# ait-detectmate/DetectMateService

Hardware: AMD Instinct MI355X
Metric: lines_per_sec (higher is better)
Workload: dtype bf16; 1 GPU; model=matcher_parser+new_value+bert-tiny-detector, global_batch=65536, seq_len=64, max_line_len=256, parallelism=dp1, ingest=shm_ring+proto_decode, transformer=True, hip_graph=False, device=cuda:0

## Files before the change

### detectmateservice_amd/ops/csrc/bert_fused.hip

```cpp
#include "common.h"
#include "kernels.h"

typedef __attribute__((address_space(3))) short lds_short;
typedef __attribute__((address_space(3))) short4v lds_short4;
typedef __attribute__((address_space(3))) float lds_float;
typedef __attribute__((address_space(1))) const short glob_cshort;
typedef __attribute__((address_space(1))) const float glob_cfloat;

#define BF_THREADS (BF_WAVES * DMX_WAVE)

#define XS (BF_H + 8)
#define QKS (2 * BF_H + 16)
#define VTS (BF_S + 8)

extern __shared__ __attribute__((aligned(16))) short smem_raw[];

template <int OFF_, int ROWS, int COLS_, int STRIDE_>
struct Tile {
  static constexpr int OFF = OFF_, COLS = COLS_, STRIDE = STRIDE_;
  static constexpr int END = OFF + ROWS * STRIDE;
  static_assert(OFF % 4 == 0 && STRIDE % 4 == 0 && COLS <= STRIDE,
                "8-byte LDS access: offsets and strides are multiples of 4");
  static __device__ __forceinline__ lds_short* ptr() {
    return (lds_short*)smem_raw + OFF;
  }
};
using XTile = Tile<0, BF_S, BF_H, XS>;
using QkTile = Tile<XTile::END, BF_S, 2 * BF_H, QKS>;
using PTiles = Tile<XTile::END, BF_WAVES * 16, BF_S, VTS>;
using AttnOut = Tile<PTiles::END, BF_S, BF_H, XS>;
using FfnHalf = Tile<XTile::END, BF_S, BF_FFN / 2, QKS>;
using VtTile = Tile<AttnOut::END, 2 * BF_DH, BF_S, VTS>;
using XMid = Tile<VtTile::OFF, BF_S, BF_H, XS>;
constexpr int RED_OFF = VtTile::END;

static_assert(QkTile::END <= VtTile::OFF, "Q|K runs past buf");
static_assert(FfnHalf::END <= VtTile::OFF, "the FFN half runs past buf");
static_assert(PTiles::END <= AttnOut::OFF,
              "the P tiles reach into the attention output");
static_assert(AttnOut::END <= VtTile::OFF,
              "the attention output runs past buf");
static_assert(XMid::END <= VtTile::END, "XMid runs past vt");
static_assert(BF_LDS_BYTES == RED_OFF * sizeof(short) + BF_H * sizeof(float),
              "kernels.h BF_LDS_BYTES out of step with the LDS strides");
static_assert(FB_BQKV % 4 == 0 && FB_BO % 4 == 0 && FB_B1 % 4 == 0 &&
                  FB_B2 % 4 == 0 && FB_SIZE % 4 == 0 &&
                  (BF_FFN / 2) % 4 == 0,
              "16-byte bias loads: bias offsets must be multiples of 4");

struct FragLane {
  int l15, l4;
  __device__ __forceinline__ explicit FragLane(int lane)
      : l15(lane & 15), l4(lane >> 4) {}
};

static __device__ __forceinline__ bf16x8 lds_frag(const lds_short* base,
                                                  int stride, int r0, int k0,
                                                  FragLane fl) {
  return *(const __attribute__((address_space(3))) bf16x8*)(
      base + (r0 + fl.l15) * stride + k0 + fl.l4 * 8);
}

static __device__ __forceinline__ lds_short4* lds_quad(lds_short* base,
                                                       int stride, int r0,
                                                       int c0, FragLane fl) {
  return (lds_short4*)(base + (r0 + fl.l15) * stride + c0 + fl.l4 * 4);
}

typedef __attribute__((ext_vector_type(4))) __bf16 bf16x4_t;
static __device__ __forceinline__ short4v pack_bf16x4(f32x4 v) {
  return __builtin_bit_cast(short4v, __builtin_convertvector(v, bf16x4_t));
}

template <int K, int MODE, int ACT, int WTS, int ABL, bool BIAS, bool SWAP>
static __device__ __forceinline__ void gemm_quad(
    const lds_short* __restrict__ in_lds, int in_stride,
    const glob_cshort* __restrict__ Wt, const glob_cfloat* __restrict__ bias,
    lds_short* __restrict__ out_lds, int out_stride,
    lds_short* __restrict__ x_lds, lds_short* __restrict__ vt_lds, int fn,
    int lane, bf16x8 zb) {
  static_assert(SWAP || MODE == 1, "only the V quads keep weight-as-B order");
  constexpr int KS = K / 32;
  const int l15 = lane & 15;
  const int l4 = lane >> 4;
  f32x4 binit = {0.f, 0.f, 0.f, 0.f};
  if constexpr (BIAS) {
    if constexpr (SWAP) {
      binit = *(const __attribute__((address_space(1))) f32x4*)(bias + fn * 16 +
                                                               l4 * 4);
    } else {
      const float bval = bias[fn * 16 + l15];
      binit = {bval, bval, bval, bval};
    }
  }
  f32x4 acc[4];
#pragma unroll
  for (int i = 0; i < 4; ++i) acc[i] = binit;
#pragma unroll 4
  for (int ks = 0; ks < KS; ++ks) {
    bf16x8 w;
    if constexpr (ABL & 1) {
      w = zb;
    } else {
      w = *(const __attribute__((address_space(1))) bf16x8*)(
          Wt + (long)(fn * 16 + l15) * WTS + ks * 32 + l4 * 8);
    }
#pragma unroll
    for (int fm = 0; fm < 4; ++fm) {
      bf16x8 a;
      if constexpr (ABL & 2) {
        a = zb;
      } else {
        a = *(const __attribute__((address_space(3))) bf16x8*)(
            in_lds + (fm * 16 + l15) * in_stride + ks * 32 + l4 * 8);
      }
      if constexpr (SWAP)
        acc[fm] = __builtin_amdgcn_mfma_f32_16x16x32_bf16(w, a, acc[fm], 0, 0, 0);
      else
        acc[fm] = __builtin_amdgcn_mfma_f32_16x16x32_bf16(a, w, acc[fm], 0, 0, 0);
    }
  }
#pragma unroll
  for (int fm = 0; fm < 4; ++fm) {
    f32x4 v = acc[fm];
    if constexpr (!SWAP) {
      *(lds_short4*)(vt_lds + (fn * 16 + l15 - 2 * BF_H) * VTS + fm * 16 +
                     l4 * 4) = pack_bf16x4(v);
    } else if constexpr (MODE == 2) {
      lds_short4* px = (lds_short4*)(x_lds + (fm * 16 + l15) * XS + fn * 16 + l4 * 4);
      const short4v xv = *px;
#pragma unroll
      for (int r = 0; r < 4; ++r) v[r] += bf16_to_f32(xv[r]);
      *px = pack_bf16x4(v);
    } else if constexpr (MODE == 3) {
      const int off = (fm * 16 + l15) * XS + fn * 16 + l4 * 4;
      const short4v xv = *(const lds_short4*)(x_lds + off);
#pragma unroll
      for (int r = 0; r < 4; ++r) v[r] += bf16_to_f32(xv[r]);
      *(lds_short4*)(out_lds + off) = pack_bf16x4(v);
    } else {
      if constexpr (ACT == 1) {
#pragma unroll
        for (int r = 0; r < 4; ++r) v[r] = gelu_f32(v[r]);
      }
      *(lds_short4*)(out_lds + (fm * 16 + l15) * out_stride + fn * 16 + l4 * 4) =
          pack_bf16x4(v);
    }
  }
}

template <int K, int MODE, int ACT, int WTS, int ABL, bool BIAS, bool SWAP,
          int CNT>
static __device__ __forceinline__ void gemm_quads(
    const lds_short* __restrict__ in_lds, int in_stride,
    const glob_cshort* __restrict__ Wt, const glob_cfloat* __restrict__ bias,
    lds_short* __restrict__ out_lds, int out_stride,
    lds_short* __restrict__ x_lds, lds_short* __restrict__ vt_lds, int fn0,
    int lane, bf16x8 zb) {
#pragma unroll 2
  for (int q = 0; q < CNT; ++q)
    gemm_quad<K, MODE, ACT, WTS, ABL, BIAS, SWAP>(in_lds, in_stride, Wt, bias, out_lds,
                                            out_stride, x_lds, vt_lds, fn0 + q,
                                            lane, zb);
}

template <int K, int N, int MODE, int ACT, int WTS, int ABL = 0,
          bool BIAS = true>
static __device__ __attribute__((noinline)) void block_gemm(
    const lds_short* __restrict__ in_lds, int in_stride,
    const glob_cshort* __restrict__ Wt, const glob_cfloat* __restrict__ bias,
    lds_short* __restrict__ out_lds, int out_stride,
    lds_short* __restrict__ x_lds, lds_short* __restrict__ vt_lds, int wid,
    int lane) {
  bf16x8 zb;
  if constexpr (ABL != 0) {
#pragma unroll
    for (int j = 0; j < 8; ++j) zb[j] = (short)0x3f01;
    asm volatile("" : "+v"(zb));
  }
  constexpr int N16 = N / 16;
  constexpr int TOTAL = 4 * N16;
  constexpr int FPW = TOTAL / BF_WAVES;
  static_assert(FPW >= 4 && FPW % 4 == 0, "quad-chunked assignment");
  constexpr int QPW = FPW / 4;
  const int fn_lo = __builtin_amdgcn_readfirstlane(wid) * QPW;
  if constexpr (MODE != 1) {
    gemm_quads<K, MODE, ACT, WTS, ABL, BIAS, true, QPW>(in_lds, in_stride, Wt, bias,
                                                  out_lds, out_stride, x_lds,
                                                  vt_lds, fn_lo, lane, zb);
  } else {
    constexpr int FN_SWAP = 2 * BF_H / 16;
    constexpr int NSW = FN_SWAP % QPW;
    if (fn_lo + QPW <= FN_SWAP) {
      gemm_quads<K, MODE, ACT, WTS, ABL, BIAS, true, QPW>(in_lds, in_stride, Wt, bias,
                                                    out_lds, out_stride, x_lds,
                                                    vt_lds, fn_lo, lane, zb);
    } else if (fn_lo >= FN_SWAP) {
      gemm_quads<K, MODE, ACT, WTS, ABL, BIAS, false, QPW>(in_lds, in_stride, Wt,
                                                     bias, out_lds, out_stride,
                                                     x_lds, vt_lds, fn_lo, lane,
                                                     zb);
    } else {
      gemm_quads<K, MODE, ACT, WTS, ABL, BIAS, true, NSW>(in_lds, in_stride, Wt, bias,
                                                    out_lds, out_stride, x_lds,
                                                    vt_lds, fn_lo, lane, zb);
      gemm_quads<K, MODE, ACT, WTS, ABL, BIAS, false, QPW - NSW>(
          in_lds, in_stride, Wt, bias, out_lds, out_stride, x_lds, vt_lds,
          fn_lo + NSW, lane, zb);
    }
  }
}

static __device__ __forceinline__ void embed(
    const unsigned char* __restrict__ lines, const int* __restrict__ start,
    const int* __restrict__ end, const short* __restrict__ wb, lds_short* x_lds,
    int line, int max_len, int tid) {
  const int s0 = start[line], e0 = end[line];
  for (int i = tid * 8; i < BF_S * BF_H; i += BF_THREADS * 8) {
    const int s = i / BF_H, c = i % BF_H;
    int tok = 0;
    const int idx = s0 + s;
    if (idx < e0 && idx < max_len)
      tok = (int)lines[(long)line * max_len + idx] + 3;
    short8v te = *(const short8v*)(wb + WB_TOK + (long)tok * BF_H + c);
    short8v pe = *(const short8v*)(wb + WB_POS + (long)s * BF_H + c);
    short8v xv;
#pragma unroll
    for (int j = 0; j < 8; ++j)
      xv[j] = f32_to_bf16(bf16_to_f32(te[j]) + bf16_to_f32(pe[j]));
    *(__attribute__((address_space(3))) short8v*)(x_lds + s * XS + c) = xv;
  }
}

static __device__ __forceinline__ void attention(int wid, int lane) {
  const FragLane fl(lane);
  const int hh = wid >> 2;
  const int q0 = (wid & 3) * 16;
  const float scale = 0.125f;

  f32x4 acc_p[4];
#pragma unroll
  for (int f = 0; f < 4; ++f) acc_p[f] = {0.f, 0.f, 0.f, 0.f};
#pragma unroll
  for (int ks = 0; ks < BF_DH / 32; ++ks) {
    bf16x8 qf = lds_frag(QkTile::ptr(), QKS, q0, hh * BF_DH + ks * 32, fl);
#pragma unroll
    for (int f = 0; f < 4; ++f)
      acc_p[f] = __builtin_amdgcn_mfma_f32_16x16x32_bf16(
          lds_frag(QkTile::ptr(), QKS, f * 16, BF_H + hh * BF_DH + ks * 32, fl),
          qf, acc_p[f], 0, 0, 0);
  }
  float m = -1e30f;
#pragma unroll
  for (int f = 0; f < 4; ++f)
#pragma unroll
    for (int r = 0; r < 4; ++r) m = fmaxf(m, acc_p[f][r] * scale);
  m = fmaxf(m, __shfl_xor(m, 16, 64));
  m = fmaxf(m, __shfl_xor(m, 32, 64));
  float sum = 0.f;
#pragma unroll
  for (int f = 0; f < 4; ++f)
#pragma unroll
    for (int r = 0; r < 4; ++r) {
      const float e = __expf(acc_p[f][r] * scale - m);
      acc_p[f][r] = e;
      sum += e;
    }
  sum += __shfl_xor(sum, 16, 64);
  sum += __shfl_xor(sum, 32, 64);
  const float inv = 1.f / sum;
  __syncthreads();
  lds_short* my_p = PTiles::ptr() + wid * 16 * VTS;
#pragma unroll
  for (int f = 0; f < 4; ++f)
    *lds_quad(my_p, VTS, 0, f * 16, fl) = pack_bf16x4(acc_p[f]);
  asm volatile("s_waitcnt lgkmcnt(0)" ::: "memory");

  f32x4 acc_o[4];
#pragma unroll
  for (int f = 0; f < 4; ++f) acc_o[f] = {0.f, 0.f, 0.f, 0.f};
#pragma unroll
  for (int ks = 0; ks < BF_S / 32; ++ks) {
    bf16x8 pf = lds_frag(my_p, VTS, 0, ks * 32, fl);
#pragma unroll
    for (int f = 0; f < 4; ++f)
      acc_o[f] = __builtin_amdgcn_mfma_f32_16x16x32_bf16(
          lds_frag(VtTile::ptr(), VTS, hh * BF_DH + f * 16, ks * 32, fl), pf,
          acc_o[f], 0, 0, 0);
  }
#pragma unroll
  for (int f = 0; f < 4; ++f) {
    f32x4 o = acc_o[f];
#pragma unroll
    for (int r = 0; r < 4; ++r) o[r] *= inv;
    *lds_quad(AttnOut::ptr(), XS, q0, hh * BF_DH + f * 16, fl) = pack_bf16x4(o);
  }
}

static __device__ __forceinline__ void block_layernorm(
    lds_short* x_lds, const short* __restrict__ gamma,
    const short* __restrict__ beta, int wid, int lane, float eps) {
  const int row = wid * 8 + (lane >> 3);
  const int c0 = (lane & 7) * 16;
  short8v va = *(const __attribute__((address_space(3))) short8v*)(x_lds + row * XS + c0);
  short8v vb = *(const __attribute__((address_space(3))) short8v*)(x_lds + row * XS + c0 + 8);
  float v[16];
  float sum = 0.f;
#pragma unroll
  for (int j = 0; j < 8; ++j) {
    v[j] = bf16_to_f32(va[j]);
    v[8 + j] = bf16_to_f32(vb[j]);
    sum += v[j] + v[8 + j];
  }
#pragma unroll
  for (int mask = 1; mask < 8; mask <<= 1) sum += __shfl_xor(sum, mask, 64);
  const float mean = sum / BF_H;
  float var = 0.f;
#pragma unroll
  for (int j = 0; j < 16; ++j) {
    const float d = v[j] - mean;
    var += d * d;
  }
#pragma unroll
  for (int mask = 1; mask < 8; mask <<= 1) var += __shfl_xor(var, mask, 64);
  const float rstd = rsqrtf(var / BF_H + eps);
  short8v ga = *(const short8v*)(gamma + c0);
  short8v gb = *(const short8v*)(gamma + c0 + 8);
  short8v ba = *(const short8v*)(beta + c0);
  short8v bb = *(const short8v*)(beta + c0 + 8);
  short8v oa, ob;
#pragma unroll
  for (int j = 0; j < 8; ++j) {
    oa[j] = f32_to_bf16((v[j] - mean) * rstd * bf16_to_f32(ga[j]) +
                        bf16_to_f32(ba[j]));
    ob[j] = f32_to_bf16((v[8 + j] - mean) * rstd * bf16_to_f32(gb[j]) +
                        bf16_to_f32(bb[j]));
  }
  *(__attribute__((address_space(3))) short8v*)(x_lds + row * XS + c0) = oa;
  *(__attribute__((address_space(3))) short8v*)(x_lds + row * XS + c0 + 8) = ob;
}

static __device__ __forceinline__ void pool_score(
    const short* __restrict__ w_score, const float* __restrict__ b_score,
    float* __restrict__ score, int tid) {
  const lds_short* x_lds = XTile::ptr();
  lds_float* red = (lds_float*)((lds_short*)smem_raw + RED_OFF);
  if (tid < BF_H) {
    float s = 0.f;
    for (int row = 0; row < BF_S; ++row)
      s += bf16_to_f32(x_lds[row * XS + tid]);
    red[tid] = (s / BF_S) * bf16_to_f32(w_score[tid]);
  }
  __syncthreads();
  const int wid = tid / DMX_WAVE, lane = tid % DMX_WAVE;
  if (wid == 0) {
    float v = red[lane] + red[lane + 64];
    v = warp_reduce_sum_f32(v);
    if (lane == 0) *score = v + *b_score;
  }
}

static __device__ __forceinline__ void pool_embed(
    float* __restrict__ emb, const float* __restrict__ mu,
    const float* __restrict__ inv_var, float* __restrict__ dist, int line,
    int tid) {
  const lds_short* x_lds = XTile::ptr();
  lds_float* red = (lds_float*)((lds_short*)smem_raw + RED_OFF);
  if (tid < BF_H) {
    float s = 0.f;
    for (int row = 0; row < BF_S; ++row)
      s += bf16_to_f32(x_lds[row * XS + tid]);
    const float m = s / BF_S;
    if (emb != nullptr) emb[(long)line * BF_H + tid] = m;
    if (mu != nullptr) {
      const float d = m - mu[tid];
      red[tid] = d * d * inv_var[tid];
    }
  }
  if (mu == nullptr) return;
  __syncthreads();
  const int wid = tid / DMX_WAVE, lane = tid % DMX_WAVE;
  if (wid == 0) {
    float v = red[lane] + red[lane + 64];
    v = warp_reduce_sum_f32(v);
    if (lane == 0) dist[line] = sqrtf(v / BF_H);
  }
}

#define HEAD_SCORE 0
#define HEAD_EMBED 1

#define PH_QKV 1
#define PH_ATTN 2
#define PH_PROJ 4
#define PH_LN 8
#define PH_FFN 16
#define PH_ALL 31

template <bool TIMED>
struct StampRecorder {
  __device__ void mark() {}
  __device__ void flush(unsigned long long*, int, int, int) {}
};
template <>
struct StampRecorder<true> {
  unsigned long long t[BF_NSTAMP];
  int n = 0;
  __device__ void mark() {
    if (n < BF_NSTAMP) t[n++] = __builtin_amdgcn_s_memrealtime();
  }
  __device__ void flush(unsigned long long* out, int line, int wid, int lane) {
    if (lane == 0 && out != nullptr) {
      unsigned long long* dst = out + ((long)line * BF_WAVES + wid) * BF_NSTAMP;
      for (int k = 0; k < BF_NSTAMP; ++k) dst[k] = k < n ? t[k] : 0ull;
    }
  }
};

template <int PHASES, bool TIMED = false, int ABL = 0, int HEAD = HEAD_SCORE>
static __device__ __forceinline__ void bert_fused_body(
    const unsigned char* __restrict__ lines,
    const int* __restrict__ start,
    const int* __restrict__ end,
    const short* __restrict__ wb,
    const float* __restrict__ fb,
    float* __restrict__ scores,
    int B, int max_len, int n_layers, float eps,
    unsigned long long* __restrict__ stamps_out = nullptr,
    float* __restrict__ emb = nullptr,
    const float* __restrict__ mu = nullptr,
    const float* __restrict__ inv_var = nullptr,
    float* __restrict__ dist = nullptr) {
  StampRecorder<TIMED> stamp;
  const int line = blockIdx.x;
  if (line >= B) return;
  const int tid = threadIdx.x;
  const int wid = tid / DMX_WAVE;
  const int lane = tid % DMX_WAVE;

  lds_short* const x = XTile::ptr();

  stamp.mark();
  embed(lines, start, end, wb, x, line, max_len, tid);
  stamp.mark();
  __syncthreads();
  stamp.mark();

  for (int layer = 0; layer < n_layers; ++layer) {
    const short* lw = wb + WB_LAYER0 + (long)layer * LW_SIZE;
    const float* lf = fb + (long)layer * FB_SIZE;

    if (PHASES & PH_QKV)
      block_gemm<BF_H, 3 * BF_H, 1, 0, BF_H, ABL>(x, XS, (glob_cshort*)(lw + LW_QKV),
                                             (glob_cfloat*)(lf + FB_BQKV), QkTile::ptr(), QKS, x, VtTile::ptr(),
                                             wid, lane);
    stamp.mark();
    __syncthreads();
    stamp.mark();

    if (PHASES & PH_ATTN) attention(wid, lane);
    stamp.mark();
    __syncthreads();
    stamp.mark();

    if (PHASES & PH_PROJ)
      block_gemm<BF_H, BF_H, 2, 0, BF_H, ABL>(AttnOut::ptr(), XS, (glob_cshort*)(lw + LW_WO),
                                         (glob_cfloat*)(lf + FB_BO), nullptr, 0, x,
                                         nullptr, wid, lane);
    __syncthreads();
    if (PHASES & PH_LN)
      block_layernorm(x, lw + LW_LN1G, lw + LW_LN1B, wid, lane, eps);
    stamp.mark();
    __syncthreads();
    stamp.mark();

    if (PHASES & PH_FFN)
#pragma unroll
    for (int h = 0; h < 2; ++h) {
      block_gemm<BF_H, BF_FFN / 2, 0, 1, BF_H, ABL>(
          x, XS, (glob_cshort*)(lw + LW_W1 + (long)h * (BF_FFN / 2) * BF_H),
          (glob_cfloat*)(lf + FB_B1 + h * (BF_FFN / 2)), FfnHalf::ptr(), QKS, nullptr,
          nullptr, wid, lane);
      __syncthreads();
      if (h == 0)
        block_gemm<BF_FFN / 2, BF_H, 3, 0, BF_FFN, ABL, true>(
            FfnHalf::ptr(), QKS, (glob_cshort*)(lw + LW_W2), (glob_cfloat*)(lf + FB_B2),
            XMid::ptr(), XS, x, nullptr, wid, lane);
      else
        block_gemm<BF_FFN / 2, BF_H, 3, 0, BF_FFN, ABL, false>(
            FfnHalf::ptr(), QKS, (glob_cshort*)(lw + LW_W2 + (long)h * (BF_FFN / 2)),
            nullptr, x, XS, XMid::ptr(), nullptr, wid, lane);
      __syncthreads();
    }
    if (PHASES & PH_LN)
      block_layernorm(x, lw + LW_LN2G, lw + LW_LN2B, wid, lane, eps);
    stamp.mark();
    __syncthreads();
    stamp.mark();
  }

  if constexpr (HEAD == HEAD_EMBED)
    pool_embed(emb, mu, inv_var, dist, line, tid);
  else
    pool_score(wb + WB_LAYER0 + (long)n_layers * LW_SIZE,
               fb + (long)n_layers * FB_SIZE, scores + line, tid);
  stamp.mark();
  stamp.flush(stamps_out, line, wid, lane);
}

extern "C" __global__ __launch_bounds__(BF_THREADS, 4)
void dmx_bert_fused_bf16(const unsigned char* __restrict__ lines,
                         const int* __restrict__ start,
                         const int* __restrict__ end,
                         const short* __restrict__ wb,
                         const float* __restrict__ fb,
                         float* __restrict__ scores, int B, int max_len,
                         int n_layers, float eps) {
  bert_fused_body<PH_ALL>(lines, start, end, wb, fb, scores, B, max_len,
                          n_layers, eps);
}

extern "C" __global__ __launch_bounds__(BF_THREADS, 4)
void dmx_bert_fused_embed_bf16(const unsigned char* __restrict__ lines,
                               const int* __restrict__ start,
                               const int* __restrict__ end,
                               const short* __restrict__ wb,
                               const float* __restrict__ fb,
                               float* __restrict__ emb,
                               const float* __restrict__ mu,
                               const float* __restrict__ inv_var,
                               float* __restrict__ dist, int B, int max_len,
                               int n_layers, float eps) {
  bert_fused_body<PH_ALL, false, 0, HEAD_EMBED>(lines, start, end, wb, fb,
                                                nullptr, B, max_len, n_layers,
                                                eps, nullptr, emb, mu, inv_var,
                                                dist);
}

template <int PHASES, int ABL = 0>
__global__ __launch_bounds__(BF_THREADS, 4) void dmx_bert_fused_probe(
    const unsigned char* lines, const int* start, const int* end,
    const short* wb, const float* fb, float* scores, int B, int max_len,
    int n_layers, float eps) {
  bert_fused_body<PHASES, false, ABL>(lines, start, end, wb, fb, scores, B,
                                      max_len, n_layers, eps);
}

extern "C" __global__ __launch_bounds__(BF_THREADS, 4)
void dmx_bert_fused_timed(const unsigned char* lines, const int* start,
                          const int* end, const short* wb, const float* fb,
                          float* scores, int B, int max_len, int n_layers,
                          float eps, unsigned long long* stamps) {
  bert_fused_body<PH_ALL, true>(lines, start, end, wb, fb, scores, B,
                                max_len, n_layers, eps, stamps);
}

constexpr int BF_MAX_DEVICES = 64;
typedef bool AttrDone[BF_MAX_DEVICES];

template <typename... KArgs, typename... Args>
static hipError_t launch_bert_fused(void (*kernel)(KArgs...),
                                    AttrDone& attr_done, int B,
                                    hipStream_t stream, Args... args) {
  int dev = 0;
  hipError_t err = hipGetDevice(&dev);
  if (err != hipSuccess) return err;
  if (dev < 0 || dev >= BF_MAX_DEVICES) return hipErrorInvalidDevice;
  if (!attr_done[dev]) {
    err = hipFuncSetAttribute((const void*)kernel,
                              hipFuncAttributeMaxDynamicSharedMemorySize,
                              BF_LDS_BYTES);
    if (err != hipSuccess) return err;
    attr_done[dev] = true;
  }
  hipLaunchKernelGGL(kernel, dim3(B), dim3(BF_THREADS), BF_LDS_BYTES, stream,
                     args...);
  return hipSuccess;
}

extern "C" hipError_t dmx_launch_bert_fused_bf16(
    const uint8_t* lines, const int32_t* start, const int32_t* end,
    const int16_t* wb, const float* fb, float* scores, int B, int max_len,
    int n_layers, float eps, hipStream_t stream) {
  static AttrDone attr_done;
  return launch_bert_fused(dmx_bert_fused_bf16, attr_done, B, stream, lines,
                           start, end, wb, fb, scores, B, max_len, n_layers,
                           eps);
}

extern "C" hipError_t dmx_launch_bert_fused_embed(
    const uint8_t* lines, const int32_t* start, const int32_t* end,
    const int16_t* wb, const float* fb, float* emb, const float* mu,
    const float* inv_var, float* dist, int B, int max_len, int n_layers,
    float eps, hipStream_t stream) {
  static AttrDone attr_done;
  return launch_bert_fused(dmx_bert_fused_embed_bf16, attr_done, B, stream,
                           lines, start, end, wb, fb, emb, mu, inv_var, dist,
                           B, max_len, n_layers, eps);
}

extern "C" hipError_t dmx_launch_bert_fused_timed(
    const uint8_t* lines, const int32_t* start, const int32_t* end,
    const int16_t* wb, const float* fb, float* scores, int64_t* stamps, int B,
    int max_len, int n_layers, float eps, hipStream_t stream) {
  static AttrDone attr_done;
  return launch_bert_fused(dmx_bert_fused_timed, attr_done, B, stream, lines,
                           start, end, wb, fb, scores, B, max_len, n_layers,
                           eps, (unsigned long long*)stamps);
}

struct ProbeVariant {
  int mask;
  decltype(&dmx_bert_fused_probe<0, 0>) kernel;
  AttrDone attr_done;
};
template <int PHASES, int ABL = 0>
constexpr ProbeVariant probe_variant() {
  return {PHASES | (ABL << 8), dmx_bert_fused_probe<PHASES, ABL>, {}};
}
static ProbeVariant probe_variants[] = {
    probe_variant<0>(),
    probe_variant<PH_QKV>(),
    probe_variant<PH_QKV | PH_ATTN>(),
    probe_variant<PH_QKV | PH_ATTN | PH_PROJ>(),
    probe_variant<PH_QKV | PH_ATTN | PH_PROJ | PH_LN>(),
    probe_variant<PH_ALL>(),
    probe_variant<PH_FFN>(),
    probe_variant<PH_LN>(),
    probe_variant<PH_ALL, 1>(),
    probe_variant<PH_ALL, 2>(),
    probe_variant<PH_ALL, 3>(),
    probe_variant<PH_FFN, 1>(),
    probe_variant<PH_FFN, 2>(),
    probe_variant<PH_FFN, 3>(),
};

static ProbeVariant* find_probe_variant(int phase_mask) {
  for (ProbeVariant& v : probe_variants)
    if (v.mask == phase_mask) return &v;
  return nullptr;
}

extern "C" bool dmx_bert_fused_probe_mask_known(int phase_mask) {
  return find_probe_variant(phase_mask) != nullptr;
}

extern "C" hipError_t dmx_launch_bert_fused_probe(
    const uint8_t* lines, const int32_t* start, const int32_t* end,
    const int16_t* wb, const float* fb, float* scores, int B, int max_len,
    int n_layers, float eps, int phase_mask, hipStream_t stream) {
  ProbeVariant* v = find_probe_variant(phase_mask);
  if (v == nullptr) return hipErrorInvalidValue;
  return launch_bert_fused(v->kernel, v->attr_done, B, stream, lines, start,
                           end, wb, fb, scores, B, max_len, n_layers, eps);
}
```

Baseline: 8.571 million lines/s.

## Keep activation fragments stationary in registers across quads for K=128 GEMMs

Adds an activation-stationary GEMM path for the K=128 projections. It loads the 4x4 activation fragments from LDS once per wave and reuses them across all of the wave's output quads, and it prefetches the next quad's weights and bias while the current MFMAs run. By default this is enabled only for the fused QKV GEMM; the W1 path stays on the old routine because its macro defaults to off. The change also re-materialises lane and wave ids per layer to steer register allocation. Holding the fragments costs more VGPRs, which may hurt occupancy under the 4-blocks-per-CU launch bound.

```diff
diff --git a/detectmateservice_amd/ops/csrc/bert_fused.hip b/detectmateservice_amd/ops/csrc/bert_fused.hip
--- a/detectmateservice_amd/ops/csrc/bert_fused.hip
+++ b/detectmateservice_amd/ops/csrc/bert_fused.hip
@@ -162,6 +162,118 @@
     gemm_quad<K, MODE, ACT, WTS, ABL, BIAS, SWAP>(in_lds, in_stride, Wt, bias, out_lds,
                                             out_stride, x_lds, vt_lds, fn0 + q,
                                             lane, zb);
+}
+
+#ifndef BF_ASTAT_QKV
+#define BF_ASTAT_QKV 1
+#endif
+#ifndef BF_ASTAT_W1
+#define BF_ASTAT_W1 0
+#endif
+
+template <int WTS, int ABL>
+static __device__ __forceinline__ bf16x8 astat_wfrag(
+    const glob_cshort* __restrict__ Wt, int fn, int ks, int l15, int l4,
+    bf16x8 zb) {
+  if constexpr (ABL & 1) {
+    return zb;
+  } else {
+    return *(const __attribute__((address_space(1))) bf16x8*)(
+        Wt + (long)(fn * 16 + l15) * WTS + ks * 32 + l4 * 8);
+  }
+}
+
+template <bool SWAP>
+static __device__ __forceinline__ f32x4 astat_bias(
+    const glob_cfloat* __restrict__ bias, int fn, int l15, int l4) {
+  if constexpr (SWAP) {
+    return *(const __attribute__((address_space(1))) f32x4*)(bias + fn * 16 +
+                                                             l4 * 4);
+  } else {
+    const float bval = bias[fn * 16 + l15];
+    return f32x4{bval, bval, bval, bval};
+  }
+}
+
+template <int MODE, int ACT, int WTS, int ABL, int CNT, int NSW, int Q = 0>
+static __device__ __forceinline__ void astat_quads(
+    const bf16x8 (&a)[4][4], bf16x8 (&w)[4], f32x4 binit,
+    const glob_cshort* __restrict__ Wt, const glob_cfloat* __restrict__ bias,
+    lds_short* __restrict__ out_lds, int out_stride,
+    lds_short* __restrict__ vt_lds, int fn0, int lane, bf16x8 zb) {
+  constexpr bool SWAP = Q < NSW;
+  constexpr bool MORE = Q + 1 < CNT;
+  static_assert(SWAP || MODE == 1, "only the V quads keep weight-as-B order");
+  const int l15 = lane & 15;
+  const int l4 = lane >> 4;
+  const int fn = fn0 + Q;
+  f32x4 bnext = {0.f, 0.f, 0.f, 0.f};
+  if constexpr (MORE) bnext = astat_bias<(Q + 1 < NSW)>(bias, fn + 1, l15, l4);
+  f32x4 acc[4];
+#pragma unroll
+  for (int i = 0; i < 4; ++i) acc[i] = binit;
+#pragma unroll
+  for (int ks = 0; ks < 4; ++ks) {
+#pragma unroll
+    for (int fm = 0; fm < 4; ++fm) {
+      if constexpr (SWAP)
+        acc[fm] = __builtin_amdgcn_mfma_f32_16x16x32_bf16(w[ks], a[ks][fm], acc[fm], 0, 0, 0);
+      else
+        acc[fm] = __builtin_amdgcn_mfma_f32_16x16x32_bf16(a[ks][fm], w[ks], acc[fm], 0, 0, 0);
+    }
+    if constexpr (MORE) {
+      w[ks] = astat_wfrag<WTS, ABL>(Wt, fn + 1, ks, l15, l4, zb);
+      __builtin_amdgcn_sched_barrier(0);
+    }
+  }
+#pragma unroll
+  for (int fm = 0; fm < 4; ++fm) {
+    f32x4 v = acc[fm];
+    if constexpr (!SWAP) {
+      *(lds_short4*)(vt_lds + (fn * 16 + l15 - 2 * BF_H) * VTS + fm * 16 +
+                     l4 * 4) = pack_bf16x4(v);
+    } else {
+      if constexpr (ACT == 1) {
+#pragma unroll
+        for (int r = 0; r < 4; ++r) v[r] = gelu_f32(v[r]);
+      }
+      *(lds_short4*)(out_lds + (fm * 16 + l15) * out_stride + fn * 16 + l4 * 4) =
+          pack_bf16x4(v);
+    }
+  }
+  if constexpr (MORE)
+    astat_quads<MODE, ACT, WTS, ABL, CNT, NSW, Q + 1>(
+        a, w, bnext, Wt, bias, out_lds, out_stride, vt_lds, fn0, lane, zb);
+}
+
+template <int MODE, int ACT, int WTS, int ABL, int CNT, int NSW>
+static __device__ __forceinline__ void gemm_quads_astat(
+    const lds_short* __restrict__ in_lds, int in_stride,
+    const glob_cshort* __restrict__ Wt, const glob_cfloat* __restrict__ bias,
+    lds_short* __restrict__ out_lds, int out_stride,
+    lds_short* __restrict__ vt_lds, int fn0, int lane, bf16x8 zb) {
+  const int l15 = lane & 15;
+  const int l4 = lane >> 4;
+  const f32x4 binit = astat_bias<(0 < NSW)>(bias, fn0, l15, l4);
+  bf16x8 w[4];
+#pragma unroll
+  for (int ks = 0; ks < 4; ++ks)
+    w[ks] = astat_wfrag<WTS, ABL>(Wt, fn0, ks, l15, l4, zb);
+  bf16x8 a[4][4];
+#pragma unroll
+  for (int ks = 0; ks < 4; ++ks)
+#pragma unroll
+    for (int fm = 0; fm < 4; ++fm) {
+      if constexpr (ABL & 2) {
+        a[ks][fm] = zb;
+      } else {
+        a[ks][fm] = *(const __attribute__((address_space(3))) bf16x8*)(
+            in_lds + (fm * 16 + l15) * in_stride + ks * 32 + l4 * 8);
+      }
+    }
+  __builtin_amdgcn_sched_barrier(0);
+  astat_quads<MODE, ACT, WTS, ABL, CNT, NSW>(a, w, binit, Wt, bias, out_lds,
+                                             out_stride, vt_lds, fn0, lane, zb);
 }
 
 template <int K, int N, int MODE, int ACT, int WTS, int ABL = 0,
@@ -211,6 +323,51 @@
   }
 }
 
+template <int N, int MODE, int ACT, int ABL>
+static __device__ __forceinline__ void block_gemm_k128(
+    const lds_short* __restrict__ in_lds, int in_stride,
+    const glob_cshort* __restrict__ Wt, const glob_cfloat* __restrict__ bias,
+    lds_short* __restrict__ out_lds, int out_stride,
+    lds_short* __restrict__ vt_lds, int wid, int lane) {
+  static_assert(MODE == 0 || MODE == 1, "the multi-quad K = 128 GEMMs");
+  constexpr int QPW = N / 16 / BF_WAVES;
+  static_assert(QPW > 1 && QPW * 16 * BF_WAVES == N, "whole quads per wave");
+  if constexpr (MODE == 1 ? !BF_ASTAT_QKV : !BF_ASTAT_W1) {
+    block_gemm<BF_H, N, MODE, ACT, BF_H, ABL>(in_lds, in_stride, Wt, bias,
+                                              out_lds, out_stride, nullptr,
+                                              vt_lds, wid, lane);
+  } else {
+    bf16x8 zb;
+    if constexpr (ABL != 0) {
+#pragma unroll
+      for (int j = 0; j < 8; ++j) zb[j] = (short)0x3f01;
+      asm volatile("" : "+v"(zb));
+    }
+    const int fn_lo = __builtin_amdgcn_readfirstlane(wid) * QPW;
+    if constexpr (MODE == 0) {
+      gemm_quads_astat<MODE, ACT, BF_H, ABL, QPW, QPW>(
+          in_lds, in_stride, Wt, bias, out_lds, out_stride, vt_lds, fn_lo, lane,
+          zb);
+    } else {
+      constexpr int FN_SWAP = 2 * BF_H / 16;
+      constexpr int NSW = FN_SWAP % QPW;
+      if (fn_lo + QPW <= FN_SWAP) {
+        gemm_quads_astat<MODE, ACT, BF_H, ABL, QPW, QPW>(
+            in_lds, in_stride, Wt, bias, out_lds, out_stride, vt_lds, fn_lo,
+            lane, zb);
+      } else if (fn_lo >= FN_SWAP) {
+        gemm_quads_astat<MODE, ACT, BF_H, ABL, QPW, 0>(
+            in_lds, in_stride, Wt, bias, out_lds, out_stride, vt_lds, fn_lo,
+            lane, zb);
+      } else {
+        gemm_quads_astat<MODE, ACT, BF_H, ABL, QPW, NSW>(
+            in_lds, in_stride, Wt, bias, out_lds, out_stride, vt_lds, fn_lo,
+            lane, zb);
+      }
+    }
+  }
+}
+
 static __device__ __forceinline__ void embed(
     const unsigned char* __restrict__ lines, const int* __restrict__ start,
     const int* __restrict__ end, const short* __restrict__ wb, lds_short* x_lds,
@@ -435,8 +592,8 @@
   const int line = blockIdx.x;
   if (line >= B) return;
   const int tid = threadIdx.x;
-  const int wid = tid / DMX_WAVE;
-  const int lane = tid % DMX_WAVE;
+  const int wid0 = tid / DMX_WAVE;
+  const int lane0 = tid % DMX_WAVE;
 
   lds_short* const x = XTile::ptr();
 
@@ -449,11 +606,13 @@
   for (int layer = 0; layer < n_layers; ++layer) {
     const short* lw = wb + WB_LAYER0 + (long)layer * LW_SIZE;
     const float* lf = fb + (long)layer * FB_SIZE;
+    int lane = lane0, wid = wid0;
+    asm volatile("" : "+v"(lane), "+v"(wid));
 
     if (PHASES & PH_QKV)
-      block_gemm<BF_H, 3 * BF_H, 1, 0, BF_H, ABL>(x, XS, (glob_cshort*)(lw + LW_QKV),
-                                             (glob_cfloat*)(lf + FB_BQKV), QkTile::ptr(), QKS, x, VtTile::ptr(),
-                                             wid, lane);
+      block_gemm_k128<3 * BF_H, 1, 0, ABL>(x, XS, (glob_cshort*)(lw + LW_QKV),
+                                           (glob_cfloat*)(lf + FB_BQKV), QkTile::ptr(), QKS,
+                                           VtTile::ptr(), wid, lane);
     stamp.mark();
     __syncthreads();
     stamp.mark();
@@ -477,9 +636,9 @@
     if (PHASES & PH_FFN)
 #pragma unroll
     for (int h = 0; h < 2; ++h) {
-      block_gemm<BF_H, BF_FFN / 2, 0, 1, BF_H, ABL>(
+      block_gemm_k128<BF_FFN / 2, 0, 1, ABL>(
           x, XS, (glob_cshort*)(lw + LW_W1 + (long)h * (BF_FFN / 2) * BF_H),
-          (glob_cfloat*)(lf + FB_B1 + h * (BF_FFN / 2)), FfnHalf::ptr(), QKS, nullptr,
+          (glob_cfloat*)(lf + FB_B1 + h * (BF_FFN / 2)), FfnHalf::ptr(), QKS,
           nullptr, wid, lane);
       __syncthreads();
       if (h == 0)
@@ -505,7 +664,7 @@
     pool_score(wb + WB_LAYER0 + (long)n_layers * LW_SIZE,
                fb + (long)n_layers * FB_SIZE, scores + line, tid);
   stamp.mark();
-  stamp.flush(stamps_out, line, wid, lane);
+  stamp.flush(stamps_out, line, wid0, lane0);
 }
 
 extern "C" __global__ __launch_bounds__(BF_THREADS, 4)
```

Measured after the change: 7.402 million lines/s. 0.864x the previous value.

## Prefetch GEMM weights before block barriers and software-pipeline quad weight loads

Applied to the files above, without the earlier changes.

Splits the per-quad GEMM into operand load, MFMA chain and store, so that the global weight and bias loads for the first quad are issued before the preceding __syncthreads. The barrier moves inside block_gemm, letting weight fetch latency overlap the wait. Weights for the next quad are prefetched while the current quad's results are stored. The cost is higher register use, since all K/32 weight fragments are held at once under the existing 4-block launch bound, and barrier placement is reworked, which makes timing stamps shift.

```diff
diff --git a/detectmateservice_amd/ops/csrc/bert_fused.hip b/detectmateservice_amd/ops/csrc/bert_fused.hip
--- a/detectmateservice_amd/ops/csrc/bert_fused.hip
+++ b/detectmateservice_amd/ops/csrc/bert_fused.hip
@@ -72,18 +72,11 @@
   return __builtin_bit_cast(short4v, __builtin_convertvector(v, bf16x4_t));
 }
 
-template <int K, int MODE, int ACT, int WTS, int ABL, bool BIAS, bool SWAP>
-static __device__ __forceinline__ void gemm_quad(
-    const lds_short* __restrict__ in_lds, int in_stride,
+template <int K, int WTS, int ABL, bool BIAS, bool SWAP>
+static __device__ __forceinline__ void quad_operands(
     const glob_cshort* __restrict__ Wt, const glob_cfloat* __restrict__ bias,
-    lds_short* __restrict__ out_lds, int out_stride,
-    lds_short* __restrict__ x_lds, lds_short* __restrict__ vt_lds, int fn,
-    int lane, bf16x8 zb) {
-  static_assert(SWAP || MODE == 1, "only the V quads keep weight-as-B order");
-  constexpr int KS = K / 32;
-  const int l15 = lane & 15;
-  const int l4 = lane >> 4;
-  f32x4 binit = {0.f, 0.f, 0.f, 0.f};
+    int fn, int l15, int l4, bf16x8 zb, bf16x8 (&w)[K / 32], f32x4& binit) {
+  binit = {0.f, 0.f, 0.f, 0.f};
   if constexpr (BIAS) {
     if constexpr (SWAP) {
       binit = *(const __attribute__((address_space(1))) f32x4*)(bias + fn * 16 +
@@ -93,18 +86,25 @@
       binit = {bval, bval, bval, bval};
     }
   }
-  f32x4 acc[4];
-#pragma unroll
-  for (int i = 0; i < 4; ++i) acc[i] = binit;
-#pragma unroll 4
+#pragma unroll
+  for (int ks = 0; ks < K / 32; ++ks) {
+    if constexpr (ABL & 1) {
+      w[ks] = zb;
+    } else {
+      w[ks] = *(const __attribute__((address_space(1))) bf16x8*)(
+          Wt + (long)(fn * 16 + l15) * WTS + ks * 32 + l4 * 8);
+    }
+  }
+  __builtin_amdgcn_sched_barrier(0);
+}
+
+template <int K, int ABL, bool SWAP>
+static __device__ __forceinline__ void quad_chain(
+    const lds_short* __restrict__ in_lds, int in_stride, int l15, int l4,
+    bf16x8 zb, const bf16x8 (&w)[K / 32], f32x4 (&acc)[4]) {
+  constexpr int KS = K / 32;
+#pragma unroll
   for (int ks = 0; ks < KS; ++ks) {
-    bf16x8 w;
-    if constexpr (ABL & 1) {
-      w = zb;
-    } else {
-      w = *(const __attribute__((address_space(1))) bf16x8*)(
-          Wt + (long)(fn * 16 + l15) * WTS + ks * 32 + l4 * 8);
-    }
 #pragma unroll
     for (int fm = 0; fm < 4; ++fm) {
       bf16x8 a;
@@ -115,11 +115,19 @@
             in_lds + (fm * 16 + l15) * in_stride + ks * 32 + l4 * 8);
       }
       if constexpr (SWAP)
-        acc[fm] = __builtin_amdgcn_mfma_f32_16x16x32_bf16(w, a, acc[fm], 0, 0, 0);
+        acc[fm] = __builtin_amdgcn_mfma_f32_16x16x32_bf16(w[ks], a, acc[fm], 0, 0, 0);
       else
-        acc[fm] = __builtin_amdgcn_mfma_f32_16x16x32_bf16(a, w, acc[fm], 0, 0, 0);
-    }
-  }
+        acc[fm] = __builtin_amdgcn_mfma_f32_16x16x32_bf16(a, w[ks], acc[fm], 0, 0, 0);
+    }
+  }
+}
+
+template <int MODE, int ACT, bool SWAP>
+static __device__ __forceinline__ void quad_store(
+    lds_short* __restrict__ out_lds, int out_stride,
+    lds_short* __restrict__ x_lds, lds_short* __restrict__ vt_lds, int fn,
+    int l15, int l4, const f32x4 (&acc)[4]) {
+  static_assert(SWAP || MODE == 1, "only the V quads keep weight-as-B order");
 #pragma unroll
   for (int fm = 0; fm < 4; ++fm) {
     f32x4 v = acc[fm];
@@ -150,28 +158,50 @@
 }
 
 template <int K, int MODE, int ACT, int WTS, int ABL, bool BIAS, bool SWAP,
-          int CNT>
+          int CNT, bool BAR, typename... REC>
 static __device__ __forceinline__ void gemm_quads(
     const lds_short* __restrict__ in_lds, int in_stride,
     const glob_cshort* __restrict__ Wt, const glob_cfloat* __restrict__ bias,
     lds_short* __restrict__ out_lds, int out_stride,
     lds_short* __restrict__ x_lds, lds_short* __restrict__ vt_lds, int fn0,
-    int lane, bf16x8 zb) {
-#pragma unroll 2
-  for (int q = 0; q < CNT; ++q)
-    gemm_quad<K, MODE, ACT, WTS, ABL, BIAS, SWAP>(in_lds, in_stride, Wt, bias, out_lds,
-                                            out_stride, x_lds, vt_lds, fn0 + q,
-                                            lane, zb);
+    int lane, bf16x8 zb, REC&... rec) {
+  const int l15 = lane & 15;
+  const int l4 = lane >> 4;
+  bf16x8 w[K / 32];
+  f32x4 binit;
+  quad_operands<K, WTS, ABL, BIAS, SWAP>(Wt, bias, fn0, l15, l4, zb, w, binit);
+  unsigned long long crossed = 0;
+  if constexpr (BAR) {
+    __syncthreads();
+    if constexpr (sizeof...(REC) != 0) {
+      crossed = __builtin_amdgcn_s_memrealtime();
+      asm volatile("" : "+s"(crossed));
+    }
+    __builtin_amdgcn_sched_barrier(0);
+  }
+#pragma unroll
+  for (int q = 0; q < CNT; ++q) {
+    f32x4 acc[4];
+#pragma unroll
+    for (int i = 0; i < 4; ++i) acc[i] = binit;
+    quad_chain<K, ABL, SWAP>(in_lds, in_stride, l15, l4, zb, w, acc);
+    if (q + 1 < CNT)
+      quad_operands<K, WTS, ABL, BIAS, SWAP>(Wt, bias, fn0 + q + 1, l15, l4,
+                                             zb, w, binit);
+    quad_store<MODE, ACT, SWAP>(out_lds, out_stride, x_lds, vt_lds, fn0 + q,
+                                l15, l4, acc);
+  }
+  if constexpr (BAR) (rec.mark_at(crossed), ...);
 }
 
 template <int K, int N, int MODE, int ACT, int WTS, int ABL = 0,
-          bool BIAS = true>
+          bool BIAS = true, bool BAR = false, typename... REC>
 static __device__ __attribute__((noinline)) void block_gemm(
     const lds_short* __restrict__ in_lds, int in_stride,
     const glob_cshort* __restrict__ Wt, const glob_cfloat* __restrict__ bias,
     lds_short* __restrict__ out_lds, int out_stride,
     lds_short* __restrict__ x_lds, lds_short* __restrict__ vt_lds, int wid,
-    int lane) {
+    int lane, REC&... rec) {
   bf16x8 zb;
   if constexpr (ABL != 0) {
 #pragma unroll
@@ -185,26 +215,25 @@
   constexpr int QPW = FPW / 4;
   const int fn_lo = __builtin_amdgcn_readfirstlane(wid) * QPW;
   if constexpr (MODE != 1) {
-    gemm_quads<K, MODE, ACT, WTS, ABL, BIAS, true, QPW>(in_lds, in_stride, Wt, bias,
-                                                  out_lds, out_stride, x_lds,
-                                                  vt_lds, fn_lo, lane, zb);
+    gemm_quads<K, MODE, ACT, WTS, ABL, BIAS, true, QPW, BAR>(
+        in_lds, in_stride, Wt, bias, out_lds, out_stride, x_lds, vt_lds, fn_lo,
+        lane, zb, rec...);
   } else {
     constexpr int FN_SWAP = 2 * BF_H / 16;
     constexpr int NSW = FN_SWAP % QPW;
     if (fn_lo + QPW <= FN_SWAP) {
-      gemm_quads<K, MODE, ACT, WTS, ABL, BIAS, true, QPW>(in_lds, in_stride, Wt, bias,
-                                                    out_lds, out_stride, x_lds,
-                                                    vt_lds, fn_lo, lane, zb);
+      gemm_quads<K, MODE, ACT, WTS, ABL, BIAS, true, QPW, BAR>(
+          in_lds, in_stride, Wt, bias, out_lds, out_stride, x_lds, vt_lds,
+          fn_lo, lane, zb, rec...);
     } else if (fn_lo >= FN_SWAP) {
-      gemm_quads<K, MODE, ACT, WTS, ABL, BIAS, false, QPW>(in_lds, in_stride, Wt,
-                                                     bias, out_lds, out_stride,
-                                                     x_lds, vt_lds, fn_lo, lane,
-                                                     zb);
+      gemm_quads<K, MODE, ACT, WTS, ABL, BIAS, false, QPW, BAR>(
+          in_lds, in_stride, Wt, bias, out_lds, out_stride, x_lds, vt_lds,
+          fn_lo, lane, zb, rec...);
     } else {
-      gemm_quads<K, MODE, ACT, WTS, ABL, BIAS, true, NSW>(in_lds, in_stride, Wt, bias,
-                                                    out_lds, out_stride, x_lds,
-                                                    vt_lds, fn_lo, lane, zb);
-      gemm_quads<K, MODE, ACT, WTS, ABL, BIAS, false, QPW - NSW>(
+      gemm_quads<K, MODE, ACT, WTS, ABL, BIAS, true, NSW, BAR>(
+          in_lds, in_stride, Wt, bias, out_lds, out_stride, x_lds, vt_lds,
+          fn_lo, lane, zb, rec...);
+      gemm_quads<K, MODE, ACT, WTS, ABL, BIAS, false, QPW - NSW, false>(
           in_lds, in_stride, Wt, bias, out_lds, out_stride, x_lds, vt_lds,
           fn_lo + NSW, lane, zb);
     }
@@ -406,8 +435,9 @@
 struct StampRecorder<true> {
   unsigned long long t[BF_NSTAMP];
   int n = 0;
-  __device__ void mark() {
-    if (n < BF_NSTAMP) t[n++] = __builtin_amdgcn_s_memrealtime();
+  __device__ void mark() { mark_at(__builtin_amdgcn_s_memrealtime()); }
+  __device__ void mark_at(unsigned long long now) {
+    if (n < BF_NSTAMP) t[n++] = now;
   }
   __device__ void flush(unsigned long long* out, int line, int wid, int lane) {
     if (lane == 0 && out != nullptr) {
@@ -416,6 +446,24 @@
     }
   }
 };
+
+template <int K, int N, int MODE, int ACT, int WTS, int ABL, bool BIAS,
+          bool STAMPED, bool TIMED>
+static __device__ __forceinline__ void block_gemm_bar(
+    const lds_short* __restrict__ in_lds, int in_stride,
+    const glob_cshort* __restrict__ Wt, const glob_cfloat* __restrict__ bias,
+    lds_short* __restrict__ out_lds, int out_stride,
+    lds_short* __restrict__ x_lds, lds_short* __restrict__ vt_lds, int wid,
+    int lane, StampRecorder<TIMED>& stamp) {
+  if constexpr (STAMPED && TIMED)
+    block_gemm<K, N, MODE, ACT, WTS, ABL, BIAS, true>(
+        in_lds, in_stride, Wt, bias, out_lds, out_stride, x_lds, vt_lds, wid,
+        lane, stamp);
+  else
+    block_gemm<K, N, MODE, ACT, WTS, ABL, BIAS, true>(
+        in_lds, in_stride, Wt, bias, out_lds, out_stride, x_lds, vt_lds, wid,
+        lane);
+}
 
 template <int PHASES, bool TIMED = false, int ABL = 0, int HEAD = HEAD_SCORE>
 static __device__ __forceinline__ void bert_fused_body(
@@ -443,61 +491,75 @@
   stamp.mark();
   embed(lines, start, end, wb, x, line, max_len, tid);
   stamp.mark();
-  __syncthreads();
-  stamp.mark();
 
   for (int layer = 0; layer < n_layers; ++layer) {
     const short* lw = wb + WB_LAYER0 + (long)layer * LW_SIZE;
     const float* lf = fb + (long)layer * FB_SIZE;
 
-    if (PHASES & PH_QKV)
-      block_gemm<BF_H, 3 * BF_H, 1, 0, BF_H, ABL>(x, XS, (glob_cshort*)(lw + LW_QKV),
-                                             (glob_cfloat*)(lf + FB_BQKV), QkTile::ptr(), QKS, x, VtTile::ptr(),
-                                             wid, lane);
+    if (PHASES & PH_QKV) {
+      block_gemm_bar<BF_H, 3 * BF_H, 1, 0, BF_H, ABL, true, true, TIMED>(
+          x, XS, (glob_cshort*)(lw + LW_QKV), (glob_cfloat*)(lf + FB_BQKV),
+          QkTile::ptr(), QKS, x, VtTile::ptr(), wid, lane, stamp);
+    } else {
+      __syncthreads();
+      stamp.mark();
+    }
     stamp.mark();
     __syncthreads();
     stamp.mark();
 
     if (PHASES & PH_ATTN) attention(wid, lane);
     stamp.mark();
-    __syncthreads();
-    stamp.mark();
-
-    if (PHASES & PH_PROJ)
-      block_gemm<BF_H, BF_H, 2, 0, BF_H, ABL>(AttnOut::ptr(), XS, (glob_cshort*)(lw + LW_WO),
-                                         (glob_cfloat*)(lf + FB_BO), nullptr, 0, x,
-                                         nullptr, wid, lane);
+
+    if (PHASES & PH_PROJ) {
+      block_gemm_bar<BF_H, BF_H, 2, 0, BF_H, ABL, true, true, TIMED>(
+          AttnOut::ptr(), XS, (glob_cshort*)(lw + LW_WO),
+          (glob_cfloat*)(lf + FB_BO), nullptr, 0, x, nullptr, wid, lane, stamp);
+    } else {
+      __syncthreads();
+      stamp.mark();
+    }
     __syncthreads();
     if (PHASES & PH_LN)
       block_layernorm(x, lw + LW_LN1G, lw + LW_LN1B, wid, lane, eps);
     stamp.mark();
-    __syncthreads();
-    stamp.mark();
-
-    if (PHASES & PH_FFN)
-#pragma unroll
-    for (int h = 0; h < 2; ++h) {
-      block_gemm<BF_H, BF_FFN / 2, 0, 1, BF_H, ABL>(
-          x, XS, (glob_cshort*)(lw + LW_W1 + (long)h * (BF_FFN / 2) * BF_H),
-          (glob_cfloat*)(lf + FB_B1 + h * (BF_FFN / 2)), FfnHalf::ptr(), QKS, nullptr,
-          nullptr, wid, lane);
+
+    if (PHASES & PH_FFN) {
+#pragma unroll
+      for (int h = 0; h < 2; ++h) {
+        const glob_cshort* w1 =
+            (glob_cshort*)(lw + LW_W1 + (long)h * (BF_FFN / 2) * BF_H);
+        const glob_cfloat* b1 = (glob_cfloat*)(lf + FB_B1 + h * (BF_FFN / 2));
+        if (h == 0) {
+          block_gemm_bar<BF_H, BF_FFN / 2, 0, 1, BF_H, ABL, true, true, TIMED>(
+              x, XS, w1, b1, FfnHalf::ptr(), QKS, nullptr, nullptr, wid, lane,
+              stamp);
+          block_gemm_bar<BF_FFN / 2, BF_H, 3, 0, BF_FFN, ABL, true, false,
+                         TIMED>(FfnHalf::ptr(), QKS, (glob_cshort*)(lw + LW_W2),
+                                (glob_cfloat*)(lf + FB_B2), XMid::ptr(), XS, x,
+                                nullptr, wid, lane, stamp);
+        } else {
+          block_gemm_bar<BF_H, BF_FFN / 2, 0, 1, BF_H, ABL, true, false, TIMED>(
+              x, XS, w1, b1, FfnHalf::ptr(), QKS, nullptr, nullptr, wid, lane,
+              stamp);
+          block_gemm_bar<BF_FFN / 2, BF_H, 3, 0, BF_FFN, ABL, false, false,
+                         TIMED>(
+              FfnHalf::ptr(), QKS,
+              (glob_cshort*)(lw + LW_W2 + (long)h * (BF_FFN / 2)), nullptr, x,
+              XS, XMid::ptr(), nullptr, wid, lane, stamp);
+        }
+      }
       __syncthreads();
-      if (h == 0)
-        block_gemm<BF_FFN / 2, BF_H, 3, 0, BF_FFN, ABL, true>(
-            FfnHalf::ptr(), QKS, (glob_cshort*)(lw + LW_W2), (glob_cfloat*)(lf + FB_B2),
-            XMid::ptr(), XS, x, nullptr, wid, lane);
-      else
-        block_gemm<BF_FFN / 2, BF_H, 3, 0, BF_FFN, ABL, false>(
-            FfnHalf::ptr(), QKS, (glob_cshort*)(lw + LW_W2 + (long)h * (BF_FFN / 2)),
-            nullptr, x, XS, XMid::ptr(), nullptr, wid, lane);
+    } else {
       __syncthreads();
+      stamp.mark();
     }
     if (PHASES & PH_LN)
       block_layernorm(x, lw + LW_LN2G, lw + LW_LN2B, wid, lane, eps);
     stamp.mark();
-    __syncthreads();
-    stamp.mark();
-  }
+  }
+  __syncthreads();
+  stamp.mark();
 
   if constexpr (HEAD == HEAD_EMBED)
     pool_embed(emb, mu, inv_var, dist, line, tid);
```

After: 8.589 million lines/s before, 9.242 million lines/s after (median of 6 runs). +7.6%, better.
